# lyclyc52/NeRF_RPN

Hardware: AMD Instinct MI355X
Metric: scenes/sec (160^3x4 grids, VGG19-3D+FPN+RPN fwd+bwd) (higher is better)
Workload: dtype bf16; 1 GPU; configs[1]: one 160x160x160x4 rgb-sigma grid per GPU, VGG19-EF 3D + FPN + anchor RPN (OBB, 16 GT boxes per scene), fwd+bwd+clip+AdamW, random-init weights; scenes_per_gpu=1, parallelism=dp1, world_size_seen=1, backend=single process

## Files before the change

### include/nerfrpn.h

```cpp
#ifndef NERFRPN_H
#define NERFRPN_H

#include <stddef.h>
#include <stdint.h>

#ifdef __cplusplus
extern "C" {
#endif

typedef void *nrpn_stream_t;

enum nrpn_status {
  NRPN_OK = 0,
  NRPN_ERR_ARG = -1,
  NRPN_ERR_LAUNCH = -2,
  NRPN_ERR_DEVICE = -3
};

enum nrpn_dtype { NRPN_F32 = 0, NRPN_BF16 = 1 };

const char *nrpn_last_error(void);
int nrpn_abi_version(void);
int nrpn_check_device(int ordinal);

// ... 25 lines not shown
int nrpn_decode_boxes_f32(const int32_t *table, const float *deltas, const int64_t *sel, int64_t count,
                          int coder, float *boxes, nrpn_stream_t stream);
int nrpn_encode_boxes_f32(const int32_t *table, const float *gt, const int64_t *sel, int64_t count,
                          int coder, float *deltas, nrpn_stream_t stream);

int nrpn_coder_pairs_f32(const float *in, const float *anchors, int64_t count, int coder, int encode, float *out,
                         nrpn_stream_t stream);
int nrpn_head_flatten_f32(const float *head, int64_t cells, int ld, int anchors_per_cell, int dw, float *logits,
                          float *deltas, nrpn_stream_t stream);
int nrpn_head_unflatten(const float *g_logits, const float *g_deltas, int64_t cells, int ld, int anchors_per_cell, int dw,
                        const float *scale2, void *d_head, int dtype, nrpn_stream_t stream);

size_t nrpn_filter_workspace_bytes(int64_t n, int box_dim);
int nrpn_filter_candidates_f32(const float *boxes, const float *logits, const int32_t *levels,
                               const uint8_t *cand_valid, int64_t n, int box_dim, const float *h_grid_size3,
                               float min_size, float score_thresh, int fix_obb_clip, float *out_boxes,
                               float *out_scores, int32_t *out_levels, int32_t *d_count, void *workspace,
                               nrpn_stream_t stream);
int nrpn_select_kept_f32(const float *boxes, const float *scores, const int32_t *levels, const uint8_t *keep,
                         const int32_t *d_count, int64_t n, int box_dim, int post_top_n, float *out_boxes,
                         float *out_scores, float *out_levels, int32_t *d_out_count, nrpn_stream_t stream);

int nrpn_match_anchors_f32(const int32_t *table, int64_t total_anchors, const float *gt_aabb, int num_gt,
                           float fg_thresh, float bg_thresh, const float *h_ori_size3, float *labels,
                           int32_t *matched, float *workspace, nrpn_stream_t stream);
int nrpn_obb_to_aabb_f32(const float *obb, float *aabb, int64_t n, nrpn_stream_t stream);

size_t nrpn_sample_workspace_bytes(void);
int nrpn_sample_pos_neg(const float *labels, int64_t total, int max_pos, int batch, int64_t seed, void *workspace, int64_t *out_pos,
                        int64_t *out_neg, int32_t *counts, nrpn_stream_t stream);
int nrpn_rpn_sampled_loss_f32(const float *logits, const float *deltas, int dw, const float *targets,
                              const int64_t *pos, int64_t npos, const int64_t *neg, int64_t nneg, float beta,
                              float *loss2, float *g_logits, float *g_deltas, nrpn_stream_t stream);

enum { NRPN_CONV_BIAS = 1, NRPN_CONV_RELU = 2, NRPN_CONV_OUT_F32 = 4,
       NRPN_CONV_DEBUG_ALIAS_TAPS = 256, NRPN_CONV_DEBUG_NO_SYNC = 512,
       NRPN_CONV_DEBUG_STAGGER = 1024,
       NRPN_CONV_DEBUG_VARIANT = 0x3000 };
int nrpn_pack_conv_weight(const float *w_ref, int cout, int cin, int taps, int dtype, void *wp_fwd, void *wp_dgrad,
                          int rows_total, int row_offset, nrpn_stream_t stream);
int nrpn_unpack_conv_wgrad(const float *gw_packed, int cout, int cin, int taps, int rows_total, int row_offset,
                           float *gw_ref, int accumulate, int slices, nrpn_stream_t stream);
size_t nrpn_conv3d_fwd_workspace_bytes(int n, int gx, int gy, int gz, int cin, int cout, int ksize, int dtype);
int nrpn_conv3d_fwd(const void *x, const void *wp, const float *bias, void *y, int n, int gx, int gy, int gz, int cin,
                    int cout, int wrows, int ksize, int dtype, int flags, void *workspace, const void *relu_mask,
                    nrpn_stream_t stream);
enum { NRPN_TILE_AUTO = 0, NRPN_TILE_128 = 128, NRPN_TILE_256X128_WS = 256, NRPN_TILE_256X256 = 512, NRPN_TILE_256X256_W4 = 1024,
       NRPN_TILE_HALO = 2048  };
typedef struct nrpn_conv_opts {
  int32_t size;
  int32_t tile;
  int32_t lds_dma;
  int32_t kstep_bytes;
  int32_t stagger;
  int32_t big_split;
  int32_t debug;
  int32_t halo_pairing;
  const float *scale;
  const void *relu_mask;
  float *stats;
} nrpn_conv_opts;
int nrpn_conv3d_fwd_ex(const void *x, const void *wp, const float *bias, void *y, int n, int gx, int gy, int gz, int cin,
                       int cout, int wrows, int ksize, int dtype, int flags, void *workspace, const nrpn_conv_opts *opts,
                       nrpn_stream_t stream);
size_t nrpn_conv3d_fwd_workspace_bytes_ex(int n, int gx, int gy, int gz, int cin, int cout, int ksize, int dtype,
                                          const nrpn_conv_opts *opts);
// ... 325 lines not shown
```

### nerf_rpn_amd/csrc/postproc.hip

```cpp
#include "geometry.cuh"

#include <algorithm>
#include <cfloat>
#include <cstring>
#include <map>
#include <mutex>
#include <utility>

thread_local char g_nrpn_err[512] = "";

int nrpn_fail(int code, const char *fmt, ...) {
  va_list ap;
  va_start(ap, fmt);
  vsnprintf(g_nrpn_err, sizeof(g_nrpn_err), fmt, ap);
  va_end(ap);
  return code;
}

extern "C" const char *nrpn_last_error(void) { return g_nrpn_err; }

int nrpn_ensure_dynamic_lds(const void *kernel, int bytes) {
  static std::mutex mu;
  static std::map<std::pair<const void *, int>, int> granted;
  int dev = 0;
// ... 1271 lines not shown
extern "C" size_t nrpn_sample_workspace_bytes(void) { return (size_t)kSampInts * 4 + (size_t)2 * kSampCap * 8; }

extern "C" int nrpn_sample_pos_neg(const float *labels, int64_t total, int max_pos, int batch, int64_t seed, void *workspace, int64_t *out_pos,
                                   int64_t *out_neg, int32_t *counts, nrpn_stream_t stream) {
  NRPN_REQUIRE(total > 0 && total < (1ll << 31), "sample: total=%lld outside (0, 2^31)", (long long)total);
  NRPN_REQUIRE(max_pos >= 0 && batch >= max_pos && batch <= kSampCap, "sample: need 0 <= max_pos <= batch <= %d (got %d, %d)", kSampCap, max_pos, batch);
  NRPN_REQUIRE(labels && workspace && out_pos && out_neg && counts, "sample: null pointer");
  hipStream_t st = as_stream(stream);
  int *ws = reinterpret_cast<int *>(workspace);
  unsigned long long *boundary = reinterpret_cast<unsigned long long *>(ws + kSampInts);
  NRPN_HIP(hipMemsetAsync(ws, 0, (size_t)kSampInts * 4, st));
  NRPN_HIP(hipMemsetAsync(counts, 0, 3 * 4, st));
  const unsigned blocks = (unsigned)std::min<int64_t>(cdiv64(total, 256 * 8), 2048);
  const uint64_t useed = (uint64_t)seed;
  hipLaunchKernelGGL(sample_hist_kernel, dim3(blocks), dim3(256), 0, st, labels, total, useed, ws);
  hipLaunchKernelGGL(sample_threshold_kernel, dim3(1), dim3(1024), 0, st, ws, max_pos, batch);
  hipLaunchKernelGGL(sample_collect_kernel, dim3(blocks), dim3(256), 0, st, labels, total, useed, ws, boundary, out_pos, out_neg);
  hipLaunchKernelGGL(sample_finish_kernel, dim3(2), dim3(1024), 0, st, ws, boundary, out_pos, out_neg, counts);
  NRPN_LAUNCH_CHECK("sample_pos_neg");
  return NRPN_OK;
}

__device__ __forceinline__ float block_sum_256(float v, float *sh) {
  for (int off = 32; off > 0; off >>= 1) v += __shfl_down(v, off, 64);
  const int w = threadIdx.x >> 6, l = threadIdx.x & 63;
  if (l == 0) sh[w] = v;
  __syncthreads();
  float r = 0.f;
  if (threadIdx.x == 0) for (int i = 0; i < (int)(blockDim.x >> 6); ++i) r += sh[i];
  __syncthreads();
  return r;
}

__global__ void __launch_bounds__(256)
sampled_loss_kernel(const float *__restrict__ logits, const float *__restrict__ deltas, int dw, const float *__restrict__ targets,
                    const int64_t *__restrict__ pos, int64_t npos, const int64_t *__restrict__ neg, int64_t nneg, float beta,
                    float *__restrict__ loss2, float *__restrict__ g_logits, float *__restrict__ g_deltas) {
  __shared__ float sh[4];
  const int64_t ns = npos + nneg;
  const float inv = 1.0f / (float)ns;
  float bce = 0.f, reg = 0.f;
  for (int64_t i = threadIdx.x; i < ns; i += blockDim.x) {
    const bool is_pos = i < npos;
    const int64_t r = is_pos ? pos[i] : neg[i - npos];
    const float x = logits[r], y = is_pos ? 1.f : 0.f;
    bce += fmaxf(x, 0.f) - x * y + log1pf(expf(-fabsf(x)));
    if (g_logits) g_logits[r] = (1.0f / (1.0f + expf(-x)) - y) * inv;
  }
  for (int64_t i = threadIdx.x; i < npos * dw; i += blockDim.x) {
    const int64_t p = i / dw;
    const int k = (int)(i - p * dw);
    const int64_t r = pos[p];
    const float d = deltas[r * dw + k] - targets[p * dw + k];
    const float ad = fabsf(d);
    reg += (ad < beta) ? 0.5f * d * d / beta : ad - 0.5f * beta;
    if (g_deltas) g_deltas[r * dw + k] = ((ad < beta) ? d / beta : (d > 0.f ? 1.f : (d < 0.f ? -1.f : 0.f))) * inv;
  }
  const float b = block_sum_256(bce, sh);
  const float g = block_sum_256(reg, sh);
  if (threadIdx.x == 0) { loss2[0] = b * inv; loss2[1] = g * inv; }
}

extern "C" int nrpn_rpn_sampled_loss_f32(const float *logits, const float *deltas, int dw, const float *targets, const int64_t *pos,
                                         int64_t npos, const int64_t *neg, int64_t nneg, float beta, float *loss2, float *g_logits,
                                         float *g_deltas, nrpn_stream_t stream) {
  NRPN_REQUIRE(dw == 6 || dw == 8, "sampled loss: dw must be 6 or 8 (got %d)", dw);
  NRPN_REQUIRE(npos >= 0 && nneg >= 0 && npos + nneg > 0, "sampled loss: empty sample");
  NRPN_REQUIRE(logits && deltas && loss2 && (npos == 0 || (pos && targets)) && (nneg == 0 || neg), "sampled loss: null pointer");
  hipLaunchKernelGGL(sampled_loss_kernel, dim3(1), dim3(256), 0, as_stream(stream), logits, deltas, dw, targets, pos, npos, neg, nneg,
                     beta, loss2, g_logits, g_deltas);
  NRPN_LAUNCH_CHECK("sampled_loss");
  return NRPN_OK;
}

constexpr int kRecallMaxGt = 1024;
__global__ void __launch_bounds__(256) recall_match_kernel(float *__restrict__ ov, int P, int G, float *__restrict__ covered) {
  __shared__ float cmax[kRecallMaxGt];
  __shared__ int carg[kRecallMaxGt];
  __shared__ int pick[2];
  const int tid = threadIdx.x, lane = tid & 63, wave = tid >> 6;
  auto scan_col = [&](int g) {
    float best = -3.0e38f;
    int arg = 0x7fffffff;
    for (int r = lane; r < P; r += 64) {
      const float v = ov[(long long)r * G + g];
      if (v > best) { best = v; arg = r; }
    }
#pragma unroll
    for (int off = 32; off > 0; off >>= 1) {
      const float ob = __shfl_xor(best, off, 64);
      const int oa = __shfl_xor(arg, off, 64);
      if (ob > best || (ob == best && oa < arg)) { best = ob; arg = oa; }
    }
    if (lane == 0) { cmax[g] = best; carg[g] = arg; }
  };
  for (int g = wave; g < G; g += 4) scan_col(g);
  __syncthreads();
  const int rounds = min(P, G);
  for (int j = 0; j < rounds; ++j) {
    if (wave == 0) {
      float best = -3.0e38f;
      int arg = 0x7fffffff;
      for (int g = lane; g < G; g += 64)
        if (cmax[g] > best) { best = cmax[g]; arg = g; }
// ... 54 lines not shown
```

### nerf_rpn_amd/model/anchor.py

```python
from typing import List, Tuple

import torch
from torch import nn, Tensor

from .. import ops
from . import hip_nn


class AnchorGenerator3D(nn.Module):
    def __init__(self, sizes, aspect_ratios, is_normalized=False):
        super().__init__()
        if is_normalized:
            raise NotImplementedError("is_normalized=True is never used by run_rpn.py (normalize_aspect_ratios = False)")
        self.sizes = sizes
        self.aspect_ratios = aspect_ratios
        self.is_normalized = is_normalized
        self.aspect_ratios_unique = [ops.unique_ratio_permutations(r) for r in aspect_ratios]
        self._tables = {}

    def num_anchors_per_location(self):
        return [len(s) * len(a) for s, a in zip(self.sizes, self.aspect_ratios_unique)]

    def table(self, mesh_size, grids, device) -> "ops.AnchorTable":
        key = (tuple(mesh_size), tuple(map(tuple, grids)), str(device))
# ... 57 lines not shown
            fine = hip_nn.run_modules(self.conv, feats_cl[0])
            out0 = ops.ConvFn.apply(fine, self._pack, self.head_rows, False, True, 2, self.cls_logits.weight, self.bbox_pred.weight,
                                    self.cls_logits.bias, self.bbox_pred.bias)
            x, segs = hip_nn.ragged_cat(feats_cl[1:])
            mods = list(self.conv)
            for i in range(0, len(mods), 2):
                x = hip_nn.conv3d(mods[i], x, relu=True, segs=segs)
            h = ops.ConvFn.apply(x, self._pack, self.head_rows, False, True, 2, self.cls_logits.weight, self.bbox_pred.weight,
                                 self.cls_logits.bias, self.bbox_pred.bias)
            return [out0] + hip_nn.ragged_split(h, feats_cl[1:])
        outs = []
        convs = [m for m in self.conv if isinstance(m, nn.Conv3d)]
        for f in feats_cl:
            t = f
            for i, cv in enumerate(convs):
                chain = ops.CHAIN_GRAD_PREMASKED | (ops.CHAIN_MASK_INPUT_GRAD if i > 0 else 0)
                t = hip_nn.conv3d(cv, t, relu=True, chain=chain)
            out_chain = ops.CHAIN_MASK_INPUT_GRAD if convs else 0
            outs.append(ops.ConvFn.apply(t, self._pack, self.head_rows, ops.ConvMode(chain=out_chain), True, 2, self.cls_logits.weight,
                                         self.bbox_pred.weight, self.cls_logits.bias, self.bbox_pred.bias))
        return outs

    def cone_depth(self):
        mods = list(self.conv)
        if len(mods) % 2:
            return None
        for i in range(0, len(mods), 2):
            cv = mods[i]
            if not (isinstance(cv, nn.Conv3d) and cv.kernel_size == (3, 3, 3) and cv.stride == (1, 1, 1) and cv.padding == (1, 1, 1)
                    and cv.in_channels == cv.out_channels and isinstance(mods[i + 1], nn.ReLU)):
                return None
        return max(len(mods) // 2 - 1, 0)

    def forward_cone(self, feats_cl: List[Tensor], plan):
        convs = [m for m in self.conv if isinstance(m, nn.Conv3d)]
        return ops.ConeHeadFn.apply(plan, self, self.num_anchors, self.delta_width, *feats_cl, *[c.weight for c in convs], *[c.bias for c in convs],
                                    self.cls_logits.weight, self.bbox_pred.weight, self.cls_logits.bias, self.bbox_pred.bias)

    def forward(self, x: List[Tensor]) -> Tuple[List[Tensor], List[Tensor]]:
        dt = x[0].dtype
        fused = self.forward_fused([hip_nn.as_ndhwc(f, dt) for f in x])
        A, dw = self.num_anchors, self.delta_width
        logits = [hip_nn.as_ncdhw(h[..., :A]) for h in fused]
        bbox = [hip_nn.as_ncdhw(h[..., A:A + A * dw]) for h in fused]
        return logits, bbox
```

### nerf_rpn_amd/model/rpn.py

```python
from typing import Dict, List, Optional, Tuple

import numpy as np
import torch
import torch.nn.functional as F
from torch import nn, Tensor

from .. import ops
from . import hip_nn
from .anchor import AnchorGenerator3D
from .coder import AABBCoder, MidpointOffsetCoder
from .coder.misc import obb2hbb_3d, obb2points_3d
from .rotated_iou.oriented_iou_loss import cal_diou_3d, cal_giou_3d, cal_iou_3d
from .utils import BalancedPositiveNegativeSampler, Matcher


def permute_and_flatten(layer: Tensor, N: int, A: int, C: int, W: int, H: int, D: int) -> Tensor:
    return layer.view(N, -1, C, W, H, D).permute(0, 3, 4, 5, 1, 2).reshape(N, -1, C)


_VIEW_CACHE = {}


def _view_stack(res, device):
    key = (float(res), str(device))
# ... 164 lines not shown
                ops.cone_from_indices(cone, pos.to(device), neg.to(device), table)
        else:
            hook = None if cone is None else (lambda op_, on_, cnt_: (ops.cone_build(cone, op_, on_, cnt_, table), cone.finish))
            pairs, flags = self.fg_bg_sampler.sample_batch(labels, pending_flags, hook)
            if n == 1:
                pos, neg = pairs[0]
            else:
                pos, neg = torch.cat([p + i * T for i, (p, _) in enumerate(pairs)]), torch.cat([q + i * T for i, (_, q) in enumerate(pairs)])
        pos, neg = pos.to(device), neg.to(device)
        if self.sampler_hook is not None or n > 1:
            pos, neg = pos.sort()[0], neg.sort()[0]
        pos, neg = pos.contiguous(), neg.contiguous()
        if n > 1:
            scene = torch.div(pos, T, rounding_mode="floor")
            local = (pos - scene * T).contiguous()
            gt_rows = []
            for i, gt in enumerate(targets):
                sel = scene == i
                if gt.numel() == 0:
                    gt_rows.append(torch.zeros((int(sel.sum()), self.num_bbox_digits), dtype=torch.float32, device=device))
                else:
                    gt_rows.append(gt.float()[matched[i][local[sel]].long()])
            matched_gt = torch.cat(gt_rows).contiguous()
        else:
            local = pos
            gt = targets[0]
            matched_gt = (gt.float()[matched[0][local].long()] if gt.numel()
                          else torch.zeros((pos.numel(), self.num_bbox_digits), dtype=torch.float32, device=device)).contiguous()
        reg_targets = ops.encode_boxes(table, matched_gt, local, int(self.rotate))
        anchors_pos = ops.anchors(table, local)
        return dict(mesh_size=tuple(mesh_size), grids=[tuple(g) for g in grids], table=table, pad=pad, labels=labels, matched=matched,
                    flags=flags, pos=pos, neg=neg, matched_gt=matched_gt, reg_targets=reg_targets, anchors_pos=anchors_pos, cone=cone)

    def compute_loss(self, prep, logits, deltas, max_mesh_dim):
        pos, neg, matched_gt = prep["pos"], prep["neg"], prep["matched_gt"]
        flat_logits, flat_deltas = logits.reshape(-1), deltas.reshape(-1, self.num_delta_digits)
        loss_obj, loss_reg_l1 = ops.SampledLossFn.apply(flat_logits, flat_deltas, prep["reg_targets"], pos, neg, 1.0 / 9)
        need_box_grad = self.rotated_iou_loss is not None or self.loss_2d_requires_grad
        if need_box_grad:
            pred_pos = self.box_coder.decode_single_diff(flat_deltas[pos], prep["anchors_pos"])
        else:
            pred_pos = self.box_coder.decode_single(flat_deltas[pos], prep["anchors_pos"])
        if self.rotated_iou_loss is not None:
            loss_reg = self.rotated_iou_loss(pred_pos, matched_gt) / (pos.numel() + neg.numel())
        else:
            loss_reg = loss_reg_l1
        with torch.set_grad_enabled(self.loss_2d_requires_grad and torch.is_grad_enabled()):
            loss_2d = self._projection_loss(pred_pos if self.loss_2d_requires_grad else pred_pos.detach(), matched_gt, max_mesh_dim)
        self.last_aux = dict(pos=pos, neg=neg, labels=prep["labels"])
        return loss_obj, loss_reg, loss_2d

    def _projection_loss(self, pred, target, max_mesh_dim):
        M, K = _view_stack(max_mesh_dim, pred.device)
        if pred.is_cuda and not (pred.requires_grad and torch.is_grad_enabled()):
            return ops.projection_loss(pred, target, M, K, 1.0 / 9, float(max_mesh_dim))
        if target.size(1) == 6:
            p = torch.cat([pred[:, :3], pred[:, 3:]], dim=0)
            t = torch.cat([target[:, :3], target[:, 3:]], dim=0)
        else:
            p, t = obb2points_3d(pred), obb2points_3d(target)
        npts = p.shape[0]
        src = torch.cat([p.float(), t.float()], dim=0)
        src = torch.cat([src, torch.ones(src.shape[0], 1, device=src.device)], dim=1)
        cam = torch.matmul(M, src.t())
        pic = torch.matmul(K, cam[:, :3])
        uv = pic[:, :2] / pic[:, 2:3]
        return F.smooth_l1_loss(uv[:, :, :npts], uv[:, :, npts:], beta=1 / 9, reduction="sum") / pred.shape[0] / max_mesh_dim

    def forward(self, meshes: Tensor, features: List[Tensor], original_mesh_sizes, targets: Optional[List[Tensor]] = None,
                objectness_output_paths=None, prepared=None):
        dt = features[0].dtype
        feats_cl = [hip_nn.as_ndhwc(f, dt) for f in features]
        n = meshes.shape[0]
        mesh_size = tuple(int(v) for v in meshes.shape[-3:])
        grids = [tuple(int(v) for v in f.shape[1:4]) for f in feats_cl]
        A, dw = self.head.num_anchors, self.num_delta_digits
        cone = prepared.get("cone") if (self.training and prepared is not None and objectness_output_paths is None
                                        and prepared["grids"] == grids and prepared["mesh_size"] == mesh_size) else None
        self.last_cone = None
        if cone is not None:
            logits, deltas = self.head.forward_cone(feats_cl, cone)
            self.last_cone = dict(rows=list(cone.counts), total_voxels=cone.total)
        else:
            heads = self.head.forward_fused(feats_cl)
            if objectness_output_paths is not None:
                self.output_objectness([hip_nn.as_ncdhw(h[..., :A]) for h in heads], original_mesh_sizes, objectness_output_paths)
            logits, deltas = ops.FlattenHeadFn.apply(A, dw, dt, *[h.reshape(n, -1, h.shape[-1]) for h in heads])
        boxes = scores = level_indexes = None
        losses = {}
        if not self.training:
            table = self.anchor_generator.table(mesh_size, grids, feats_cl[0].device)
            pad = self.anchor_generator.padding_mask(mesh_size, grids, original_mesh_sizes, logits.device) if n > 1 else None
            boxes, scores, level_indexes = self.filter_proposals(table, logits, deltas, [mesh_size] * n, pad)
            if self.record_stages:
                self.last_aux["logits"], self.last_aux["deltas"] = logits.detach(), deltas.detach()
        else:
            if targets is None:
                raise ValueError("targets should not be None")
            if prepared is None or prepared["grids"] != grids or prepared["mesh_size"] != mesh_size:
                prepared = self.prepare_targets(mesh_size, grids, targets, original_mesh_sizes, logits.device)
            lo, lr, l2 = self.compute_loss(prepared, logits, deltas, max(mesh_size))
            losses = {"loss_objectness": lo, "loss_rpn_box_reg": lr, "loss_rpn_box_reg_2d": l2}
        return boxes, level_indexes, losses, scores

    def output_objectness(self, objectness, ori_sizes, output_paths):
        for i in range(len(ori_sizes)):
            levels = {}
            for level, ob in enumerate(objectness):
                score = ob[i].float().max(dim=0)[0]
                w, l, h = np.ceil(np.array(ori_sizes[i]) / 2 ** (level + 2)).astype(int)
                levels[str(level)] = score[:w, :l, :h].cpu().numpy()
            np.savez_compressed(output_paths[i], **levels)
```

### nerf_rpn_amd/ops.py

```python
import ctypes
import itertools
import math
from collections import namedtuple
from types import SimpleNamespace

import numpy as np
import torch

from . import lib
from .lib import BF16, CONV_BIAS, CONV_OUT_F32, CONV_RELU, F32, call

_QCACHE = {"epoch": -1, "map": {}}


def query(name, *args):
    if _QCACHE["epoch"] != lib.KNOB_EPOCH[0]:
        _QCACHE["epoch"], _QCACHE["map"] = lib.KNOB_EPOCH[0], {}
    m = _QCACHE["map"]
    key = (name, args)
    v = m.get(key)
    if v is None:
        v = m[key] = lib.query(name, *args)
    return v

# ... 924 lines not shown
CONE_ENABLED = [_os.environ.get("NRPN_CONE", "1") != "0"]


class ConePlan:

    def __init__(self, grids, n_scenes, depth, device):
        self.grids = [tuple(int(v) for v in g) for g in grids]
        self.n, self.depth = int(n_scenes), int(depth)
        self.segs = [g for g in self.grids for _ in range(self.n)]
        self.nseg = len(self.segs)
        self.dims = _seg_dims(self.segs)
        self.dims_ptr = ctypes.addressof(self.dims)
        self.cells = [g[0] * g[1] * g[2] for g in self.grids]
        self.level_start = [0]
        for c in self.cells:
            self.level_start.append(self.level_start[-1] + c * self.n)
        self.total = self.level_start[-1]
        self.lists = torch.empty((self.depth + 1, self.total, 2), dtype=torch.int32, device=device)
        self.counts_dev = torch.empty(self.depth + 2, dtype=torch.int32, device=device)
        self.counts = None

    def finish(self, host):
        if host[self.depth + 1]:
            raise RuntimeError("cone_build: a sampled anchor index lies outside the anchor pyramid")
        self.counts = [int(v) for v in host[:self.depth + 1]]

    def rows(self, k):
        return self.lists[k].data_ptr(), self.counts[k]

    def tensors(self):
        return [self.lists, self.counts_dev]


def cone_from_indices(plan, pos, neg, table):
    T, n = table.total, plan.n
    ps = [(pos[(pos >= i * T) & (pos < (i + 1) * T)] - i * T).long() for i in range(n)]
    ns = [(neg[(neg >= i * T) & (neg < (i + 1) * T)] - i * T).long() for i in range(n)]
    mp, mn = max(1, max(p.numel() for p in ps)), max(1, max(q.numel() for q in ns))
    dev = plan.lists.device
    out_pos = torch.zeros((n, mp), dtype=torch.int64, device=dev)
    out_neg = torch.zeros((n, mn), dtype=torch.int64, device=dev)
    cnt = []
    for i in range(n):
        out_pos[i, :ps[i].numel()] = ps[i]
        out_neg[i, :ns[i].numel()] = ns[i]
        cnt += [ps[i].numel(), ns[i].numel(), 0]
    counts = torch.tensor(cnt, dtype=torch.int32, device=dev)
    plan.finish(cone_build(plan, out_pos, out_neg, counts, table).cpu().tolist())
    return plan


def cone_build(plan, out_pos, out_neg, counts, table):
    if table.A * sum(plan.cells) != table.total or len(table.counts) != len(plan.grids):
        raise lib.NrpnError("cone_build: the anchor table and the feature grids disagree")
    offs = (ctypes.c_int64 * (len(table.offsets)))(*[int(v) for v in table.offsets])
    ws = torch.empty(query("cone_workspace_bytes", plan.total), dtype=torch.uint8, device=out_pos.device)
    call("cone_build", _p(out_pos), _p(out_neg), _p(counts), plan.n, out_pos.shape[1], out_neg.shape[1], len(plan.grids), ctypes.addressof(offs),
         table.A, plan.dims_ptr, plan.depth, _p(plan.lists), plan.total, _p(plan.counts_dev), _p(ws), _s())
    return plan.counts_dev


def conv_rows_fwd(x, wp, bias, y, plan, k, cin, cout, wrows, ksize, flags, mask=None):
    rows, nrows = plan.rows(k)
    if nrows == 0:
        return y
    if y.dtype == torch.float32 and x.dtype == torch.bfloat16:
# ... 14 lines not shown
    dest = _WgradDest(weights, wsinks, bsinks, biases[0] is not None, rows_total)
    if nrows == 0:
        return dest.nothing()
    slices = lib.query("conv3d_wgrad_slices", 1, nrows, 1, 1, cin, rows_total, rows_total, ksize, _dt(x))
    gwp = torch.empty((slices, ksize ** 3, rows_total, cin), dtype=torch.float32, device=x.device)
    ws = torch.empty(max(256, slices * rows_total * 4), dtype=torch.uint8, device=x.device)
    call("conv3d_wgrad_rows", _p(x), _p(dy), _p(gwp), _p(dest.gb), rows, nrows, plan.nseg, plan.dims_ptr, cin, rows_total, rows_total, ksize, _dt(x),
         dest.flags, _p(ws), _s())
    return dest.deliver(gwp, slices, ws.data_ptr())


def conv_rows_wgrad_x3(x, dy, weights, biases, rows_total, ksize, plan, k, sinks=None):
    rows, nrows = plan.rows(k)
    if nrows == 0 or len(weights) != 1:
        return conv_rows_wgrad(x, dy, weights, biases, rows_total, ksize, plan, k, sinks)
    cin = x.shape[-1]
    wsinks, bsinks = sinks if sinks is not None else ([_sink(w) for w in weights], [_sink(b) for b in biases])
    dest = _WgradDest(weights, wsinks, bsinks, False, rows_total)
    xpl = split3(x, None, 2, 0b10)[1]
    dpl = split3(dy, None, 2, 0b10)[1]
    slices = lib.query("conv3d_wgrad_slices", 1, nrows, 1, 1, cin, rows_total, rows_total, ksize, BF16)
    gwp = torch.empty((3 * slices, ksize ** 3, rows_total, cin), dtype=torch.float32, device=x.device)
    ws = torch.empty(max(256, slices * rows_total * 4), dtype=torch.uint8, device=x.device)
    for j, (di, xi) in enumerate(((0, 0), (0, 1), (1, 0))):
        call("conv3d_wgrad_rows", _p(xpl[xi]), _p(dpl[di]), gwp[j * slices].data_ptr(), 0, rows, nrows, plan.nseg, plan.dims_ptr, cin, rows_total,
             rows_total, ksize, BF16, 0, _p(ws), _s())
    gw = dest.deliver(gwp, 3 * slices, 0)[0]
    return (gw, *(dest.summed_bias(dy.reshape(-1, rows_total)) if biases[0] is not None else (None,)))


class ConeHeadFn(torch.autograd.Function):

    @staticmethod
    def forward(ctx, plan, head, A, dw, *tensors):
        L = len(plan.grids)
        feats = tensors[:L]
        convs = [m for m in head.conv if isinstance(m, torch.nn.Conv3d)]
        D = len(convs)
        cw, cb = tensors[L:L + D], tensors[L + D:L + 2 * D]
        ow, ob = tensors[L + 2 * D:L + 2 * D + 2], tensors[L + 2 * D + 2:L + 2 * D + 4]
        if plan.depth != max(D - 1, 0):
            raise lib.NrpnError("ConeHeadFn: the plan must hold the lists S_0 .. S_{conv_depth - 1}")
        n, C = feats[0].shape[0], feats[0].shape[-1]
        dt = feats[0].dtype
        dev = feats[0].device
        V = plan.total
        for f in feats:
            _chk(f)
        x0 = torch.cat([f.reshape(-1, C) for f in feats], dim=0)
        if x0.shape[0] != V:
            raise lib.NrpnError("ConeHeadFn: feature maps and cone plan disagree on the voxel count")
        from .model.hip_nn import _pack_of
        hs, ops_w = [x0], []
        need_dgrad = any(f.requires_grad for f in feats)
        x3 = SPLIT3[0] and dt == torch.float32 and C % 32 == 0
        for i, cv in enumerate(convs):
            wp, wpd = _pack_of(cv).get([cw[i]], dt, C, True, C)
            bias = cb[i].detach().float().contiguous() if cb[i] is not None else None
            y = torch.empty((V, C), dtype=dt, device=dev)
            if x3:
                wp, wpd = _x3_weights(_pack_of(cv), [cw[i]], wp, wpd)
                conv_rows_fwd(split3(hs[-1], _ACT_I)[0], wp, bias, y, plan, D - 1 - i, 3 * C, C, C, 3, CONV_RELU)
            else:
                conv_rows_fwd(hs[-1], wp, bias, y, plan, D - 1 - i, C, C, C, 3, CONV_RELU)
            hs.append(y)
            ops_w.append(wpd)
        rows_total = head.head_rows
        wpo, wpdo = head._pack.get(list(ow), dt, rows_total, True, C)
        bias_o = head._pack.fused_bias(ob, rows_total) if ob[0] is not None else None
        out = torch.zeros((V, rows_total), dtype=torch.float32, device=dev)
        conv_rows_fwd(hs[-1], wpo, bias_o, out, plan, 0, C, rows_total, rows_total, 1, 0)
        T = sum(plan.cells) * A
        logits = torch.empty((n, T), dtype=torch.float32, device=dev)
        deltas = torch.empty((n, T, dw), dtype=torch.float32, device=dev)
        off = 0
        for l, c in enumerate(plan.cells):
            for i in range(n):
                r0 = plan.level_start[l] + i * c
                call("head_flatten_f32", _p(out[r0:r0 + c]), c, rows_total, A, dw, _p(logits[i, off:]), _p(deltas[i, off:]), _s())
            off += c * A
        ctx.save_for_backward(*hs, *ops_w, wpdo, *cw, *[b for b in cb if b is not None], *ow, *[b for b in ob if b is not None])
        ctx.meta = (plan, head, A, dw, L, D, n, C, dt, rows_total, [b is not None for b in cb], [b is not None for b in ob], need_dgrad)
        ctx.x3 = x3
        ctx.sinks = ([_sink(w) for w in cw], [_sink(b) for b in cb], [_sink(w) for w in ow], [_sink(b) for b in ob])
        return logits, deltas

    @staticmethod
    def backward(ctx, g_logits, g_deltas):
        IN_BACKWARD[0] += 1
        try:
            return ConeHeadFn._backward(ctx, g_logits, g_deltas)
        finally:
            IN_BACKWARD[0] -= 1

    @staticmethod
    def _backward(ctx, g_logits, g_deltas):
        plan, head, A, dw, L, D, n, C, dt, rows_total, has_cb, has_ob, need_dgrad = ctx.meta
        saved = list(ctx.saved_tensors)
        hs, saved = saved[:D + 1], saved[D + 1:]
        wpds, saved = saved[:D], saved[D:]
        wpdo, saved = saved[0], saved[1:]
        cw, saved = saved[:D], saved[D:]
        cb = []
        for h in has_cb:
            cb.append(saved.pop(0) if h else None)
        ow, saved = saved[:2], saved[2:]
        ob = [saved.pop(0) if h else None for h in has_ob]
        dev = hs[0].device
        V = plan.total
        g_logits, g_deltas = g_logits.contiguous(), g_deltas.contiguous()
        dout = torch.empty((V, rows_total), dtype=dt, device=dev)
        off = 0
        for l, c in enumerate(plan.cells):
            for i in range(n):
                r0 = plan.level_start[l] + i * c
                call("head_unflatten", _p(g_logits[i, off:]), _p(g_deltas[i, off:]), c, rows_total, A, dw, 0, _p(dout[r0:r0 + c]), _dt(dout), _s())
            off += c * A
        _wait_dgrad_operands()

        cws, cbs, ows, obs = ctx.sinks
        g_ow = _on_wgrad_stream(dev, [hs[D], dout, plan.lists], _sinks_cover((*ow, *ob), (*ows, *obs)),
                                lambda: conv_rows_wgrad(hs[D], dout, list(ow), list(ob), rows_total, 1, plan, 0, (ows, obs)))
        dh = torch.zeros((V, C), dtype=dt, device=dev)
        conv_rows_fwd(dout, wpdo, None, dh, plan, 0, rows_total, C, C, 1, 0, mask=hs[D] if D > 0 else None)
        g_cw, g_cb = [None] * D, [None] * D
        g_feats = [None] * L
        if D == 0 and need_dgrad:
            for l in range(L):
                g = plan.grids[l]
                g_feats[l] = dh[plan.level_start[l]:plan.level_start[l + 1]].view(n, g[0], g[1], g[2], C)
        x3 = ctx.x3
        rows_wgrad = conv_rows_wgrad_x3 if x3 else conv_rows_wgrad
        for i in range(D - 1, -1, -1):
            k = D - 1 - i
            x_i, dy_i = hs[i], dh
            res = _on_wgrad_stream(dev, [x_i, dy_i, plan.lists], _sinks_cover((cw[i], cb[i]), (cws[i], cbs[i])),
                                   lambda x_i=x_i, dy_i=dy_i, i=i, k=k: rows_wgrad(x_i, dy_i, [cw[i]], [cb[i]], C, 3, plan, k, ([cws[i]], [cbs[i]])))
            g_cw[i] = res[0]
            g_cb[i] = res[1] if len(res) > 1 else None
            dhs = split3(dh, _ACT_I)[0] if (x3 and (i > 0 or need_dgrad)) else None
            if i > 0:
                dprev = torch.zeros((V, C), dtype=dt, device=dev)
                if x3:
                    raw = torch.zeros((V, C), dtype=dt, device=dev)
                    conv_rows_fwd(dhs, wpds[i], None, raw, plan, k + 1, 3 * C, C, C, 3, 0)
                    call("relu_backward", _p(hs[i]), _p(raw), _p(dprev), raw.numel(), _dt(raw), _s())
                else:
                    conv_rows_fwd(dh, wpds[i], None, dprev, plan, k + 1, C, C, C, 3, 0, mask=hs[i])
                dh = dprev
            elif need_dgrad:
                for l, c in enumerate(plan.cells):
                    g = plan.grids[l]
                    if x3:
                        dyl = dhs[plan.level_start[l]:plan.level_start[l + 1]].view(n, g[0], g[1], g[2], 3 * C)
                        g_feats[l] = _conv_fwd(dyl, wpds[0], None, C, C, 3, 0, torch.float32)
                        continue
                    dyl = dh[plan.level_start[l]:plan.level_start[l + 1]].view(n, g[0], g[1], g[2], C)
                    g_feats[l] = _conv_fwd(dyl, wpds[0], None, C, C, 3, 0, dt)
        return (None, None, None, None, *g_feats, *g_cw, *g_cb, *g_ow)


STEM_HALO = [_os.environ.get("NRPN_STEM_HALO", "1") != "0"]


class StemFn(torch.autograd.Function):

    @staticmethod
    def forward(ctx, x, weight, bias, stride, cache, affine=None, relu=False):
        _chk(x)
        n, gx, gy, gz, _ = x.shape
        cout = weight.shape[0]
        halo = STEM_HALO[0] and bool(query("stem_halo_supported", gz, cout, stride, _dt(x)))
        key = (weight.data_ptr(), weight._version, x.dtype, _weight_epoch, halo)
        if cache.get("key") != key:
            PACK_COUNT["stem"] += 1
            wc = weight.detach().contiguous()
            if halo:
                wp = torch.empty((cout, query("stem_halo_kpad")), dtype=x.dtype, device=x.device)
                call("pack_stem_weight_halo", _p(wc), cout, _p(wp), _s())
            else:
                kpad = query("stem_kpad", _dt(x))
                wp = torch.empty((cout, kpad), dtype=x.dtype, device=x.device)
                call("pack_stem_weight", _p(wc), cout, _dt(x), _p(wp), _s())
            cache["key"], cache["wp"] = key, wp
        wp = cache["wp"]
        o = [(g - 1) // stride + 1 for g in (gx, gy, gz)]
        y = torch.empty((n, o[0], o[1], o[2], cout), dtype=x.dtype, device=x.device)
        if affine is not None:
            scale, shift = affine
            if halo:
                call("conv3d_stem_fwd_halo", _p(x), _p(wp), _p(shift), _p(scale), _p(y), n, gx, gy, gz, cout, CONV_BIAS | (CONV_RELU if relu else 0), _s())
            else:
# ... 1774 lines not shown
```

Measured before the change: 116.2 scenes/sec.

## Fuse sampled RPN loss into cone head, reading rows directly without flattening

When the cone plan is active and no box gradient is needed, the head computes the sampled BCE and smooth-L1 loss straight from the packed per-row head output. This skips the flatten into dense (n,T) logits/deltas tensors and the separate loss kernel. In backward, a new kernel writes the head gradient only for cone rows by binary-searching the sorted pos/neg lists, which replaces the per-level, per-scene unflatten launches. It also removes the zero-fill of the head output. This assumes pos and neg are sorted and that every sampled anchor lies in a cone row.

```diff
diff --git a/include/nerfrpn.h b/include/nerfrpn.h
--- a/include/nerfrpn.h
+++ b/include/nerfrpn.h
@@ -81,6 +81,15 @@
 int nrpn_rpn_sampled_loss_f32(const float *logits, const float *deltas, int dw, const float *targets,
                               const int64_t *pos, int64_t npos, const int64_t *neg, int64_t nneg, float beta,
                               float *loss2, float *g_logits, float *g_deltas, nrpn_stream_t stream);
+int nrpn_rpn_sampled_loss_rows_f32(const float *head, int ld, const int64_t *level_start, const int64_t *cells,
+                                   int levels, int n, int64_t T, int A, int dw, const float *targets,
+                                   const int64_t *pos, int64_t npos, const int64_t *neg, int64_t nneg, float beta,
+                                   float *loss2, float *g_obj_rows, float *g_reg_rows, float *deltas_pos,
+                                   nrpn_stream_t stream);
+int nrpn_head_grad_rows(void *d_head, int dtype, int ld, const void *rows, int64_t nrows, const int64_t *level_start,
+                        const int64_t *cells, int levels, int n, int64_t T, int A, int dw, const int64_t *pos,
+                        int64_t npos, const int64_t *neg, int64_t nneg, const float *g_obj_rows,
+                        const float *g_reg_rows, const float *s_obj, const float *s_reg, nrpn_stream_t stream);
 
 enum { NRPN_CONV_BIAS = 1, NRPN_CONV_RELU = 2, NRPN_CONV_OUT_F32 = 4,
        NRPN_CONV_DEBUG_ALIAS_TAPS = 256, NRPN_CONV_DEBUG_NO_SYNC = 512,
diff --git a/nerf_rpn_amd/csrc/postproc.hip b/nerf_rpn_amd/csrc/postproc.hip
--- a/nerf_rpn_amd/csrc/postproc.hip
+++ b/nerf_rpn_amd/csrc/postproc.hip
@@ -1327,6 +1327,17 @@
   return r;
 }
 
+__device__ __forceinline__ float bce_logits_term(float x, float y) { return fmaxf(x, 0.f) - x * y + log1pf(expf(-fabsf(x))); }
+__device__ __forceinline__ float bce_logits_grad(float x, float y, float inv) { return (1.0f / (1.0f + expf(-x)) - y) * inv; }
+__device__ __forceinline__ float smooth_l1_term(float d, float beta) {
+  const float ad = fabsf(d);
+  return (ad < beta) ? 0.5f * d * d / beta : ad - 0.5f * beta;
+}
+__device__ __forceinline__ float smooth_l1_grad(float d, float beta, float inv) {
+  const float ad = fabsf(d);
+  return ((ad < beta) ? d / beta : (d > 0.f ? 1.f : (d < 0.f ? -1.f : 0.f))) * inv;
+}
+
 __global__ void __launch_bounds__(256)
 sampled_loss_kernel(const float *__restrict__ logits, const float *__restrict__ deltas, int dw, const float *__restrict__ targets,
                     const int64_t *__restrict__ pos, int64_t npos, const int64_t *__restrict__ neg, int64_t nneg, float beta,
@@ -1339,17 +1350,16 @@
     const bool is_pos = i < npos;
     const int64_t r = is_pos ? pos[i] : neg[i - npos];
     const float x = logits[r], y = is_pos ? 1.f : 0.f;
-    bce += fmaxf(x, 0.f) - x * y + log1pf(expf(-fabsf(x)));
-    if (g_logits) g_logits[r] = (1.0f / (1.0f + expf(-x)) - y) * inv;
+    bce += bce_logits_term(x, y);
+    if (g_logits) g_logits[r] = bce_logits_grad(x, y, inv);
   }
   for (int64_t i = threadIdx.x; i < npos * dw; i += blockDim.x) {
     const int64_t p = i / dw;
     const int k = (int)(i - p * dw);
     const int64_t r = pos[p];
     const float d = deltas[r * dw + k] - targets[p * dw + k];
-    const float ad = fabsf(d);
-    reg += (ad < beta) ? 0.5f * d * d / beta : ad - 0.5f * beta;
-    if (g_deltas) g_deltas[r * dw + k] = ((ad < beta) ? d / beta : (d > 0.f ? 1.f : (d < 0.f ? -1.f : 0.f))) * inv;
+    reg += smooth_l1_term(d, beta);
+    if (g_deltas) g_deltas[r * dw + k] = smooth_l1_grad(d, beta, inv);
   }
   const float b = block_sum_256(bce, sh);
   const float g = block_sum_256(reg, sh);
@@ -1365,6 +1375,161 @@
   hipLaunchKernelGGL(sampled_loss_kernel, dim3(1), dim3(256), 0, as_stream(stream), logits, deltas, dw, targets, pos, npos, neg, nneg,
                      beta, loss2, g_logits, g_deltas);
   NRPN_LAUNCH_CHECK("sampled_loss");
+  return NRPN_OK;
+}
+
+constexpr int kHeadMaxLevels = 16;
+struct HeadLevels {
+  int64_t start[kHeadMaxLevels], cells[kHeadMaxLevels], aoff[kHeadMaxLevels + 1];
+  int64_t T, V;
+  int levels, n, A, dw, ld;
+};
+
+__device__ __forceinline__ int64_t head_row_of_anchor(const HeadLevels &h, int64_t r, int &a) {
+  a = 0;
+  if (r < 0 || r >= h.T * h.n) return -1;
+  const int64_t i = r / h.T, t = r - i * h.T;
+  int l = 0;
+  while (l + 1 < h.levels && t >= h.aoff[l + 1]) ++l;
+  const int64_t u = t - h.aoff[l], cell = u / h.A;
+  a = (int)(u - cell * h.A);
+  return h.start[l] + i * h.cells[l] + cell;
+}
+
+__device__ __forceinline__ int64_t head_anchor_of_row(const HeadLevels &h, int64_t row) {
+  if (row < 0 || row >= h.V) return -1;
+  int l = 0;
+  while (l + 1 < h.levels && row >= h.start[l + 1]) ++l;
+  const int64_t u = row - h.start[l], i = u / h.cells[l], cell = u - i * h.cells[l];
+  return i * h.T + h.aoff[l] + cell * h.A;
+}
+
+__global__ void __launch_bounds__(256)
+sampled_loss_rows_kernel(const float *__restrict__ head, HeadLevels h, const float *__restrict__ targets, const int64_t *__restrict__ pos,
+                         int64_t npos, const int64_t *__restrict__ neg, int64_t nneg, float beta, float *__restrict__ loss2,
+                         float *__restrict__ g_obj_rows, float *__restrict__ g_reg_rows, float *__restrict__ deltas_pos) {
+  __shared__ float sh[4];
+  const int64_t ns = npos + nneg;
+  const float inv = 1.0f / (float)ns;
+  const int dw = h.dw;
+  float bce = 0.f, reg = 0.f;
+  for (int64_t i = threadIdx.x; i < ns; i += blockDim.x) {
+    const bool is_pos = i < npos;
+    int a;
+    const int64_t row = head_row_of_anchor(h, is_pos ? pos[i] : neg[i - npos], a);
+    float g = 0.f;
+    if (row >= 0) {
+      const float x = head[row * h.ld + a], y = is_pos ? 1.f : 0.f;
+      bce += bce_logits_term(x, y);
+      g = bce_logits_grad(x, y, inv);
+    }
+    g_obj_rows[i] = g;
+  }
+  for (int64_t i = threadIdx.x; i < npos * dw; i += blockDim.x) {
+    const int64_t p = i / dw;
+    const int k = (int)(i - p * dw);
+    int a;
+    const int64_t row = head_row_of_anchor(h, pos[p], a);
+    float v = 0.f, g = 0.f;
+    if (row >= 0) {
+      v = head[row * h.ld + h.A + a * dw + k];
+      const float d = v - targets[p * dw + k];
+      reg += smooth_l1_term(d, beta);
+      g = smooth_l1_grad(d, beta, inv);
+    }
+    deltas_pos[i] = v;
+    g_reg_rows[i] = g;
+  }
+  const float b = block_sum_256(bce, sh);
+  const float g = block_sum_256(reg, sh);
+  if (threadIdx.x == 0) { loss2[0] = b * inv; loss2[1] = g * inv; }
+}
+
+static int head_levels_fill(HeadLevels &h, const int64_t *level_start, const int64_t *cells, int levels, int n, int64_t T, int A, int dw,
+                            int ld, const char *who) {
+  NRPN_REQUIRE(level_start && cells && levels > 0 && levels <= kHeadMaxLevels && n > 0, "%s: need 1..%d levels and n > 0", who, kHeadMaxLevels);
+  NRPN_REQUIRE(dw == 6 || dw == 8, "%s: dw must be 6 or 8 (got %d)", who, dw);
+  NRPN_REQUIRE(A > 0 && A * (1 + dw) <= ld, "%s: A * (1 + dw) must fit the row (A %d, dw %d, ld %d)", who, A, dw, ld);
+  int64_t aoff = 0, row = 0;
+  for (int l = 0; l < levels; ++l) {
+    NRPN_REQUIRE(cells[l] > 0 && level_start[l] == row, "%s: level %d of the table is not packed (level, scene)-major", who, l);
+    h.start[l] = level_start[l]; h.cells[l] = cells[l]; h.aoff[l] = aoff;
+    aoff += cells[l] * A; row += cells[l] * n;
+  }
+  for (int l = levels; l < kHeadMaxLevels; ++l) { h.start[l] = row; h.cells[l] = 1; h.aoff[l] = aoff; }
+  h.aoff[kHeadMaxLevels] = aoff;
+  NRPN_REQUIRE(aoff == T, "%s: the level table holds %lld anchors per scene, T is %lld", who, (long long)aoff, (long long)T);
+  h.T = T; h.V = row; h.levels = levels; h.n = n; h.A = A; h.dw = dw; h.ld = ld;
+  return NRPN_OK;
+}
+
+extern "C" int nrpn_rpn_sampled_loss_rows_f32(const float *head, int ld, const int64_t *level_start, const int64_t *cells, int levels, int n,
+                                              int64_t T, int A, int dw, const float *targets, const int64_t *pos, int64_t npos,
+                                              const int64_t *neg, int64_t nneg, float beta, float *loss2, float *g_obj_rows,
+                                              float *g_reg_rows, float *deltas_pos, nrpn_stream_t stream) {
+  HeadLevels h;
+  if (int rc = head_levels_fill(h, level_start, cells, levels, n, T, A, dw, ld, "sampled loss rows")) return rc;
+  NRPN_REQUIRE(npos >= 0 && nneg >= 0 && npos + nneg > 0, "sampled loss rows: empty sample");
+  NRPN_REQUIRE(head && loss2 && g_obj_rows && (npos == 0 || (pos && targets && g_reg_rows && deltas_pos)) && (nneg == 0 || neg),
+               "sampled loss rows: null pointer");
+  hipLaunchKernelGGL(sampled_loss_rows_kernel, dim3(1), dim3(256), 0, as_stream(stream), head, h, targets, pos, npos, neg, nneg, beta, loss2,
+                     g_obj_rows, g_reg_rows, deltas_pos);
+  NRPN_LAUNCH_CHECK("sampled_loss_rows");
+  return NRPN_OK;
+}
+
+__device__ __forceinline__ int64_t find_sorted(const int64_t *__restrict__ a, int64_t n, int64_t v) {
+  int64_t lo = 0, hi = n;
+  while (lo < hi) {
+    const int64_t mid = (lo + hi) >> 1;
+    if (a[mid] < v) lo = mid + 1; else hi = mid;
+  }
+  return (lo < n && a[lo] == v) ? lo : -1;
+}
+
+template <typename T>
+__global__ void __launch_bounds__(128)
+head_grad_rows_kernel(T *__restrict__ d_head, const unsigned *__restrict__ rows, HeadLevels h, const int64_t *__restrict__ pos, int64_t npos,
+                      const int64_t *__restrict__ neg, int64_t nneg, const float *__restrict__ g_obj_rows, const float *__restrict__ g_reg_rows,
+                      const float *__restrict__ s_obj, const float *__restrict__ s_reg) {
+  const int64_t row = (int64_t)rows[2 * (int64_t)blockIdx.x];
+  const int64_t r0 = head_anchor_of_row(h, row);
+  if (r0 < 0) return;
+  const int per = h.A * (1 + h.dw);
+  for (int k = threadIdx.x; k < h.ld; k += blockDim.x) {
+    float v = 0.f;
+    if (k < h.A) {
+      int64_t j = find_sorted(pos, npos, r0 + k);
+      if (j < 0) { j = find_sorted(neg, nneg, r0 + k); if (j >= 0) j += npos; }
+      if (j >= 0) v = g_obj_rows[j] * s_obj[0];
+    } else if (k < per) {
+      const int a = (k - h.A) / h.dw;
+      const int64_t j = find_sorted(pos, npos, r0 + a);
+      if (j >= 0) v = g_reg_rows[j * h.dw + (k - h.A - a * h.dw)] * s_reg[0];
+    }
+    elem<T>::st(d_head + row * h.ld + k, v);
+  }
+}
+
+extern "C" int nrpn_head_grad_rows(void *d_head, int dtype, int ld, const void *rows, int64_t nrows, const int64_t *level_start,
+                                   const int64_t *cells, int levels, int n, int64_t T, int A, int dw, const int64_t *pos, int64_t npos,
+                                   const int64_t *neg, int64_t nneg, const float *g_obj_rows, const float *g_reg_rows, const float *s_obj,
+                                   const float *s_reg, nrpn_stream_t stream) {
+  HeadLevels h;
+  if (int rc = head_levels_fill(h, level_start, cells, levels, n, T, A, dw, ld, "head grad rows")) return rc;
+  NRPN_REQUIRE(dtype == NRPN_F32 || dtype == NRPN_BF16, "head grad rows: dtype must be f32 or bf16 (got %d)", dtype);
+  NRPN_REQUIRE(nrows >= 0 && nrows <= h.V && npos >= 0 && nneg >= 0, "head grad rows: bad counts");
+  if (nrows == 0) return NRPN_OK;
+  NRPN_REQUIRE(d_head && rows && g_obj_rows && s_obj && s_reg && (npos == 0 || (pos && g_reg_rows)) && (nneg == 0 || neg),
+               "head grad rows: null pointer");
+  const unsigned *list = reinterpret_cast<const unsigned *>(rows);
+  if (dtype == NRPN_F32)
+    hipLaunchKernelGGL((head_grad_rows_kernel<float>), dim3((unsigned)nrows), dim3(128), 0, as_stream(stream), (float *)d_head, list, h, pos,
+                       npos, neg, nneg, g_obj_rows, g_reg_rows, s_obj, s_reg);
+  else
+    hipLaunchKernelGGL((head_grad_rows_kernel<unsigned short>), dim3((unsigned)nrows), dim3(128), 0, as_stream(stream),
+                       (unsigned short *)d_head, list, h, pos, npos, neg, nneg, g_obj_rows, g_reg_rows, s_obj, s_reg);
+  NRPN_LAUNCH_CHECK("head_grad_rows");
   return NRPN_OK;
 }
 
diff --git a/nerf_rpn_amd/model/anchor.py b/nerf_rpn_amd/model/anchor.py
--- a/nerf_rpn_amd/model/anchor.py
+++ b/nerf_rpn_amd/model/anchor.py
@@ -113,9 +113,9 @@
                 return None
         return max(len(mods) // 2 - 1, 0)
 
-    def forward_cone(self, feats_cl: List[Tensor], plan):
+    def forward_cone(self, feats_cl: List[Tensor], plan, loss_pack=None):
         convs = [m for m in self.conv if isinstance(m, nn.Conv3d)]
-        return ops.ConeHeadFn.apply(plan, self, self.num_anchors, self.delta_width, *feats_cl, *[c.weight for c in convs], *[c.bias for c in convs],
+        return ops.ConeHeadFn.apply(plan, self, self.num_anchors, self.delta_width, loss_pack, *feats_cl, *[c.weight for c in convs], *[c.bias for c in convs],
                                     self.cls_logits.weight, self.bbox_pred.weight, self.cls_logits.bias, self.bbox_pred.bias)
 
     def forward(self, x: List[Tensor]) -> Tuple[List[Tensor], List[Tensor]]:
diff --git a/nerf_rpn_amd/model/rpn.py b/nerf_rpn_amd/model/rpn.py
--- a/nerf_rpn_amd/model/rpn.py
+++ b/nerf_rpn_amd/model/rpn.py
@@ -220,15 +220,22 @@
         return dict(mesh_size=tuple(mesh_size), grids=[tuple(g) for g in grids], table=table, pad=pad, labels=labels, matched=matched,
                     flags=flags, pos=pos, neg=neg, matched_gt=matched_gt, reg_targets=reg_targets, anchors_pos=anchors_pos, cone=cone)
 
-    def compute_loss(self, prep, logits, deltas, max_mesh_dim):
+    def need_box_grad(self):
+        return self.rotated_iou_loss is not None or self.loss_2d_requires_grad
+
+    def compute_loss(self, prep, logits, deltas, max_mesh_dim, rows_loss=None):
         pos, neg, matched_gt = prep["pos"], prep["neg"], prep["matched_gt"]
-        flat_logits, flat_deltas = logits.reshape(-1), deltas.reshape(-1, self.num_delta_digits)
-        loss_obj, loss_reg_l1 = ops.SampledLossFn.apply(flat_logits, flat_deltas, prep["reg_targets"], pos, neg, 1.0 / 9)
-        need_box_grad = self.rotated_iou_loss is not None or self.loss_2d_requires_grad
-        if need_box_grad:
-            pred_pos = self.box_coder.decode_single_diff(flat_deltas[pos], prep["anchors_pos"])
-        else:
-            pred_pos = self.box_coder.decode_single(flat_deltas[pos], prep["anchors_pos"])
+        need_box_grad = self.need_box_grad()
+        if rows_loss is not None:
+            loss_obj, loss_reg_l1, deltas_pos = rows_loss
+            pred_pos = self.box_coder.decode_single(deltas_pos, prep["anchors_pos"])
+        else:
+            flat_logits, flat_deltas = logits.reshape(-1), deltas.reshape(-1, self.num_delta_digits)
+            loss_obj, loss_reg_l1 = ops.SampledLossFn.apply(flat_logits, flat_deltas, prep["reg_targets"], pos, neg, 1.0 / 9)
+            if need_box_grad:
+                pred_pos = self.box_coder.decode_single_diff(flat_deltas[pos], prep["anchors_pos"])
+            else:
+                pred_pos = self.box_coder.decode_single(flat_deltas[pos], prep["anchors_pos"])
         if self.rotated_iou_loss is not None:
             loss_reg = self.rotated_iou_loss(pred_pos, matched_gt) / (pos.numel() + neg.numel())
         else:
@@ -266,7 +273,14 @@
         cone = prepared.get("cone") if (self.training and prepared is not None and objectness_output_paths is None
                                         and prepared["grids"] == grids and prepared["mesh_size"] == mesh_size) else None
         self.last_cone = None
-        if cone is not None:
+        rows_loss = None
+        if cone is not None and ops.CONE_ROWS_LOSS[0] and targets is not None and not self.need_box_grad():
+            table = prepared["table"]
+            pack = (prepared["reg_targets"], prepared["pos"], prepared["neg"], 1.0 / 9, table.total)
+            rows_loss = self.head.forward_cone(feats_cl, cone, pack)
+            logits = deltas = None
+            self.last_cone = dict(rows=list(cone.counts), total_voxels=cone.total)
+        elif cone is not None:
             logits, deltas = self.head.forward_cone(feats_cl, cone)
             self.last_cone = dict(rows=list(cone.counts), total_voxels=cone.total)
         else:
@@ -287,7 +301,7 @@
                 raise ValueError("targets should not be None")
             if prepared is None or prepared["grids"] != grids or prepared["mesh_size"] != mesh_size:
                 prepared = self.prepare_targets(mesh_size, grids, targets, original_mesh_sizes, logits.device)
-            lo, lr, l2 = self.compute_loss(prepared, logits, deltas, max(mesh_size))
+            lo, lr, l2 = self.compute_loss(prepared, logits, deltas, max(mesh_size), rows_loss)
             losses = {"loss_objectness": lo, "loss_rpn_box_reg": lr, "loss_rpn_box_reg_2d": l2}
         return boxes, level_indexes, losses, scores
 
diff --git a/nerf_rpn_amd/ops.py b/nerf_rpn_amd/ops.py
--- a/nerf_rpn_amd/ops.py
+++ b/nerf_rpn_amd/ops.py
@@ -980,6 +980,17 @@
         return [self.lists, self.counts_dev]
 
 
+CONE_ROWS_LOSS = [_os.environ.get("NRPN_CONE_ROWS_LOSS", "1") != "0"]
+
+
+def _head_levels(plan):
+    if getattr(plan, "_head_levels", None) is None:
+        L = len(plan.cells)
+        plan._head_levels = ((ctypes.c_int64 * L)(*plan.level_start[:L]), (ctypes.c_int64 * L)(*plan.cells))
+    start, cells = plan._head_levels
+    return ctypes.addressof(start), ctypes.addressof(cells), len(plan.cells)
+
+
 def cone_from_indices(plan, pos, neg, table):
     T, n = table.total, plan.n
     ps = [(pos[(pos >= i * T) & (pos < (i + 1) * T)] - i * T).long() for i in range(n)]
@@ -1060,7 +1071,7 @@
 class ConeHeadFn(torch.autograd.Function):
 
     @staticmethod
-    def forward(ctx, plan, head, A, dw, *tensors):
+    def forward(ctx, plan, head, A, dw, pack, *tensors):
         L = len(plan.grids)
         feats = tensors[:L]
         convs = [m for m in head.conv if isinstance(m, torch.nn.Conv3d)]
@@ -1096,9 +1107,31 @@
         rows_total = head.head_rows
         wpo, wpdo = head._pack.get(list(ow), dt, rows_total, True, C)
         bias_o = head._pack.fused_bias(ob, rows_total) if ob[0] is not None else None
-        out = torch.zeros((V, rows_total), dtype=torch.float32, device=dev)
+        out = (torch.zeros if pack is None else torch.empty)((V, rows_total), dtype=torch.float32, device=dev)
         conv_rows_fwd(hs[-1], wpo, bias_o, out, plan, 0, C, rows_total, rows_total, 1, 0)
         T = sum(plan.cells) * A
+        ctx.save_for_backward(*hs, *ops_w, wpdo, *cw, *[b for b in cb if b is not None], *ow, *[b for b in ob if b is not None])
+        ctx.meta = (plan, head, A, dw, L, D, n, C, dt, rows_total, [b is not None for b in cb], [b is not None for b in ob], need_dgrad)
+        ctx.x3 = x3
+        ctx.sinks = ([_sink(w) for w in cw], [_sink(b) for b in cb], [_sink(w) for w in ow], [_sink(b) for b in ob])
+        ctx.rows_loss = None
+        if pack is not None:
+            targets, pos, neg, beta, pack_T = pack
+            if pack_T != T or n != plan.n:
+                raise lib.NrpnError("ConeHeadFn: the loss pack and the cone plan disagree on the anchor count")
+            targets = targets.contiguous()
+            _chk(targets, pos, neg)
+            npos, nneg = pos.numel(), neg.numel()
+            loss2 = torch.empty(2, dtype=torch.float32, device=dev)
+            g_obj = torch.empty(npos + nneg, dtype=torch.float32, device=dev)
+            g_reg = torch.empty((npos, dw), dtype=torch.float32, device=dev)
+            deltas_pos = torch.empty((npos, dw), dtype=torch.float32, device=dev)
+            call("rpn_sampled_loss_rows_f32", _p(out), rows_total, *_head_levels(plan), n, T, A, dw, _p(targets), _p(pos), npos, _p(neg), nneg,
+                 float(beta), _p(loss2), _p(g_obj), _p(g_reg), _p(deltas_pos), _s())
+            ctx.rows_loss = (pos, neg, g_obj, g_reg, T)
+            ctx.mark_non_differentiable(deltas_pos)
+            ctx.set_materialize_grads(False)
+            return loss2[0], loss2[1], deltas_pos
         logits = torch.empty((n, T), dtype=torch.float32, device=dev)
         deltas = torch.empty((n, T, dw), dtype=torch.float32, device=dev)
         off = 0
@@ -1107,14 +1140,10 @@
                 r0 = plan.level_start[l] + i * c
                 call("head_flatten_f32", _p(out[r0:r0 + c]), c, rows_total, A, dw, _p(logits[i, off:]), _p(deltas[i, off:]), _s())
             off += c * A
-        ctx.save_for_backward(*hs, *ops_w, wpdo, *cw, *[b for b in cb if b is not None], *ow, *[b for b in ob if b is not None])
-        ctx.meta = (plan, head, A, dw, L, D, n, C, dt, rows_total, [b is not None for b in cb], [b is not None for b in ob], need_dgrad)
-        ctx.x3 = x3
-        ctx.sinks = ([_sink(w) for w in cw], [_sink(b) for b in cb], [_sink(w) for w in ow], [_sink(b) for b in ob])
         return logits, deltas
 
     @staticmethod
-    def backward(ctx, g_logits, g_deltas):
+    def backward(ctx, g_logits, g_deltas, _g_deltas_pos=None):
         IN_BACKWARD[0] += 1
         try:
             return ConeHeadFn._backward(ctx, g_logits, g_deltas)
@@ -1136,14 +1165,21 @@
         ob = [saved.pop(0) if h else None for h in has_ob]
         dev = hs[0].device
         V = plan.total
-        g_logits, g_deltas = g_logits.contiguous(), g_deltas.contiguous()
         dout = torch.empty((V, rows_total), dtype=dt, device=dev)
-        off = 0
-        for l, c in enumerate(plan.cells):
-            for i in range(n):
-                r0 = plan.level_start[l] + i * c
-                call("head_unflatten", _p(g_logits[i, off:]), _p(g_deltas[i, off:]), c, rows_total, A, dw, 0, _p(dout[r0:r0 + c]), _dt(dout), _s())
-            off += c * A
+        if ctx.rows_loss is not None:
+            pos, neg, g_obj, g_reg, T = ctx.rows_loss
+            s_obj, s_reg = [torch.zeros((), dtype=torch.float32, device=dev) if g is None else g.float().contiguous() for g in (g_logits, g_deltas)]
+            rows, nrows = plan.rows(0)
+            call("head_grad_rows", _p(dout), _dt(dout), rows_total, rows, nrows, *_head_levels(plan), n, T, A, dw, _p(pos), pos.numel(), _p(neg),
+                 neg.numel(), _p(g_obj), _p(g_reg), _p(s_obj), _p(s_reg), _s())
+        else:
+            g_logits, g_deltas = g_logits.contiguous(), g_deltas.contiguous()
+            off = 0
+            for l, c in enumerate(plan.cells):
+                for i in range(n):
+                    r0 = plan.level_start[l] + i * c
+                    call("head_unflatten", _p(g_logits[i, off:]), _p(g_deltas[i, off:]), c, rows_total, A, dw, 0, _p(dout[r0:r0 + c]), _dt(dout), _s())
+                off += c * A
         _wait_dgrad_operands()
 
         cws, cbs, ows, obs = ctx.sinks
@@ -1185,7 +1221,7 @@
                         continue
                     dyl = dh[plan.level_start[l]:plan.level_start[l + 1]].view(n, g[0], g[1], g[2], C)
                     g_feats[l] = _conv_fwd(dyl, wpds[0], None, C, C, 3, 0, dt)
-        return (None, None, None, None, *g_feats, *g_cw, *g_cb, *g_ow)
+        return (None, None, None, None, None, *g_feats, *g_cw, *g_cb, *g_ow)
 
 
 STEM_HALO = [_os.environ.get("NRPN_STEM_HALO", "1") != "0"]
```

New measurement: 117.5 scenes/sec (median of 6 runs). +1.1%, better.
